# sandyz1000/face-landmark-detector

Measured on AMD Instinct MI355X. Metric: faces/sec (whole node), 256x256 batch inference: fused preprocess + FCN-8 forward + softmax + top-4 landmark decode + similarity/alignment warp, higher is better.
Workload: dtype f32; 1 GPU; BASELINE configs[1]: batch=64/GPU 256x256x3 uint8 crops, fcn_8(68) vanilla encoder fp32, random-init weights (seed 2), decode top-4 thresh 0, align to 256x256; global_batch=64, parallelism=dp1

## Files before the change

### face-landmark-detector_amd/build.py

```python
from __future__ import annotations

import concurrent.futures
import hashlib
import os
import shutil
import subprocess
import sys

HERE = os.path.dirname(os.path.abspath(__file__))
ROOT = os.path.dirname(HERE)
CSRC = os.path.join(HERE, "csrc")
INCLUDE = os.path.join(ROOT, "include")
OBJ_DIR = os.path.join(HERE, "csrc", "build")
LIB_PATH = os.path.join(HERE, "libflm_hip.so")

SOURCES = [
    "flm_api.hip",
    "flm_pack.hip",
    "flm_enc1.hip",
    "flm_igemm.hip",
    "flm_igemm_bf16.hip",
    "flm_conv3_halo.hip",
    "flm_score1x1.hip",
    "flm_tail_bf16.hip",
    "flm_convt.hip",
    "flm_up3_wreg.hip",
    "flm_decode.hip",
    "flm_decode_stats.hip",
    "flm_cand.hip",
    "flm_misc.hip",
    "flm_frames.hip",
    "flm_warp_fmt.hip",
    "flm_frames_nv12.hip",
    "flm_track.hip",
    "flm_track_assoc.hip",
    "flm_quality.hip",
    "flm_track_exit.hip",
    "flm_pose.hip",
    "flm_mobile.hip",
]
FLAGS = ["--offload-arch=gfx950", "-O3", "-fPIC", "-std=c++17", "-ffp-contract=off",
         "-Wall", "-Wno-unused-function", "-I", INCLUDE, "-I", CSRC]


FILE_FLAGS = {"flm_enc1.hip": ["-mllvm", "-amdgpu-mfma-vgpr-form"]}


def _hipcc() -> str:
    for c in (shutil.which("hipcc"), "/opt/rocm/bin/hipcc"):
        if c and os.path.exists(c):
            return c
    raise RuntimeError("hipcc not found: the HIP extension cannot be built")


def _stamp(paths) -> str:
    h = hashlib.sha256()
    h.update(" ".join(FLAGS).encode())
    h.update(repr(sorted(FILE_FLAGS.items())).encode())
    for p in sorted(paths):
        with open(p, "rb") as f:
            h.update(p.encode())
            h.update(f.read())
    return h.hexdigest()


def build(force: bool = False, verbose: bool = True, extra_flags=()) -> str:
    os.makedirs(OBJ_DIR, exist_ok=True)
    headers = [os.path.join(CSRC, f) for f in os.listdir(CSRC) if f.endswith(".h")] + \
              [os.path.join(INCLUDE, f) for f in os.listdir(INCLUDE) if f.endswith(".h")]
    srcs = [os.path.join(CSRC, s) for s in SOURCES]
    stamp = _stamp(srcs + headers) + " ".join(extra_flags)
    stamp_file = os.path.join(OBJ_DIR, "stamp.txt")
    if not force and os.path.exists(LIB_PATH) and os.path.exists(stamp_file) and open(stamp_file).read() == stamp:
        return LIB_PATH
    hipcc = _hipcc()

    def compile_one(src):
        obj = os.path.join(OBJ_DIR, os.path.basename(src) + ".o")
        cmd = [hipcc, *FLAGS, *FILE_FLAGS.get(os.path.basename(src), []), *extra_flags, "-c", src, "-o", obj]
        r = subprocess.run(cmd, capture_output=True, text=True)
        if r.returncode != 0:
            raise RuntimeError("hipcc failed on %s:\n%s\n%s" % (src, r.stdout, r.stderr))
        if verbose and r.stderr.strip():
            sys.stderr.write(r.stderr)
        return obj

    with concurrent.futures.ThreadPoolExecutor(max_workers=min(8, len(srcs))) as ex:
        objs = list(ex.map(compile_one, srcs))
    cmd = [hipcc, "--offload-arch=gfx950", "-shared", "-fPIC", "-o", LIB_PATH, *objs]
    r = subprocess.run(cmd, capture_output=True, text=True)
    if r.returncode != 0:
        raise RuntimeError("link failed:\n%s\n%s" % (r.stdout, r.stderr))
    with open(stamp_file, "w") as f:
        f.write(stamp)
    if verbose:
        print("built", LIB_PATH)
    return LIB_PATH


if __name__ == "__main__":
    build(force="--force" in sys.argv)
```

### face-landmark-detector_amd/csrc/flm_api.hip

```cpp
#include <cmath>
#include <cstdarg>
#include <cstdio>
#include <cstring>

#include "flm_common.h"

namespace flm {

static thread_local char g_err[512] = "";

void set_error(const char* fmt, ...) {
  va_list ap;
  va_start(ap, fmt);
  vsnprintf(g_err, sizeof(g_err), fmt, ap);
  va_end(ap);
}

int hip_fail(hipError_t e, const char* what) {
  set_error("HIP error %d (%s) at %s", (int)e, hipGetErrorString(e), what);
  return FLM_ERR_HIP;
}

struct Knob {
  const char* key;
  std::atomic<int> value;
  bool (*valid)(int);
  const char* domain;
};
static Knob g_knobs[] = {
    {"bf16_big_tiles", {1}, nullptr, nullptr},
    {"bf16_lds_dma", {1}, nullptr, nullptr},
    {"bf16_mfma16", {1}, nullptr, nullptr},
    {"bf16_halo_mfma16", {1}, nullptr, nullptr},
    {"f32_two_level", {1}, nullptr, nullptr},
    {"f32_lean_tile", {1}, nullptr, nullptr},
    {"bf16_group_n", {0}, [](int v) { return v >= 0 && v <= 32 && !(v & (v - 1)); }, "0 or a power of two <= 32"},
    {"bf16_conv3_halo", {1}, nullptr, nullptr},
    {"bf16_score1x1", {1}, nullptr, nullptr},
    {"bf16_fused_tail", {1}, nullptr, nullptr},
    {"decode_lds_dma", {1}, nullptr, nullptr},
    {"posmajor_order", {1}, nullptr, nullptr},
    {"warp_rows", {1}, [](int v) { return v == 0 || v == 1 || v == 4; }, "0, 1 or 4"},
    {"up3_cand8", {1}, [](int v) { return v >= 0 && v <= 7; }, "in [0,7]"},
    {"up3_cand8_rows", {0}, [](int v) { return v >= 0 && v <= 8 && !(v & (v - 1)); }, "0, 1, 2, 4 or 8"},
    {"up3_wreg", {0}, [](int v) { return v == 0 || v == 1; }, "0 or 1"},
    {"f32_fc6_rows", {0}, [](int v) { return v == 0 || v == 64 || v == 128; }, "0, 64 or 128"},
};
static_assert(sizeof(g_knobs) / sizeof(g_knobs[0]) == KNOB_COUNT, "one row per KnobId");
int tuning(KnobId id) { return g_knobs[id].value.load(std::memory_order_relaxed); }
static Knob* find_knob(const char* who, const char* key) {
  for (Knob& k : g_knobs)
    if (!strcmp(k.key, key)) return &k;
  set_error("%s: unknown key '%s'", who, key);
  return nullptr;
}

struct ProfRec {
  const char* name;
  hipEvent_t a, b;
};
static ProfRec* g_prof = nullptr;
static int g_prof_cap = 0, g_prof_n = 0;
static char g_prof_filter[32] = "";

struct ProfScope {
  hipStream_t s;
  ProfRec* r;
  ProfScope(hipStream_t st, const char* name) : s(st), r(nullptr) {
    if (name && g_prof && g_prof_n < g_prof_cap && (!g_prof_filter[0] || !strcmp(g_prof_filter, name))) {
      r = &g_prof[g_prof_n++];
      r->name = name;
      (void)hipEventRecord(r->a, s);
    }
  }
  ~ProfScope() {
    if (r) (void)hipEventRecord(r->b, s);
  }
};

struct CandOpts {
  int enable, sub, cap_div;
};
static bool resolve_opts(const flm_forward_opts* o, CandOpts* c) {
  c->enable = 1;
  c->sub = 0;
  c->cap_div = 1;
  if (!o) return true;
  if (o->struct_size < sizeof(flm_forward_opts)) {
    set_error("flm_forward_opts: struct_size %u is smaller than this library's %zu (initialise with flm_forward_opts_init)",
              o->struct_size, sizeof(flm_forward_opts));
    return false;
  }
  if (o->candidate_sub_phases < 0 || o->candidate_sub_phases > 16 || o->candidate_cap_div < 1) {
    set_error("flm_forward_opts: candidate_sub_phases must be in [0,16] and candidate_cap_div >= 1");
    return false;
  }
  c->enable = o->landmark_candidates != 0;
  c->sub = o->candidate_sub_phases;
  c->cap_div = o->candidate_cap_div;
  return true;
}
static int cand_sub_for(const CandOpts& c, int n_points, bool bf16) {
  if (c.sub > 0) return c.sub;
  return n_points <= 8 ? (bf16 ? 4 : 2) : (n_points <= 15 ? 6 : 8);
}
static bool landmark_candidates_enabled(const CandOpts& c, const ConvTGeom& g, int fcn32, int decode_mode, int n_points,
                                        int oh, int ow) {
  return c.enable && !fcn32 && decode_mode == FLM_DECODE_TOPN && n_points >= 1 && n_points <= 32 &&
         convt_candidates_supported(g) && (long long)oh * ow < (1 << 17);
}

struct EncNames {
  char s[kMaxEnc][8];
  EncNames() {
    for (int i = 0; i < kMaxEnc; ++i) snprintf(s[i], sizeof(s[i]), "enc%d", i + 1);
  }
};

static size_t take(size_t& cur, size_t bytes) {
  size_t o = cur;
  cur = align_up(cur + bytes, 256);
  return o;
}

Fcn8Ws fcn8_ws_layout(int n, int h, int w, int C, int dtype, int out_mode, int decode_mode, int n_points,
                      int arch, const flm_forward_opts* opts) {
  Fcn8Ws W;
  CandOpts co;
  if (!resolve_opts(opts, &co)) {
    W = Fcn8Ws();
    W.total = 0;
    return W;
// ... 44 lines not shown
    }
  }
  W.total = cur;
  return W;
}

static int check_dtype_classes(const char* what, int dtype, int C) {
  if (dtype != FLM_F32 && dtype != FLM_BF16) {
    set_error("%s: unknown dtype %d (FLM_F32 = 0, FLM_BF16 = 1)", what, dtype);
    return FLM_ERR_UNSUPPORTED;
  }
  if (C < 1 || C > kMaxClasses) {
    set_error("%s: n_classes must be in [1,%d] (got %d)", what, kMaxClasses, C);
    return FLM_ERR_SHAPE;
  }
  return FLM_OK;
}

static int check_fcn8_shape(int n, int h, int w, int C, int dtype) {
  const int rc = check_dtype_classes("fcn8", dtype, C);
  if (rc) return rc;
  if (n <= 0 || h <= 0 || w <= 0 || (h % 32) || (w % 32)) {
    set_error("fcn8: input must be [N>0, H, W, 3] with H and W multiples of 32 (got n=%d h=%d w=%d)", n, h, w);
    return FLM_ERR_SHAPE;
  }
  if (n > (1 << 24) || h > (1 << 15) || w > (1 << 15) || (long long)n * (h + 32) * (w + 32) * C >= (1ll << 40)) {
    set_error("fcn8: batch too large (n=%d h=%d w=%d: at most 2^40 output values per call)", n, h, w);
    return FLM_ERR_SHAPE;
  }
  return FLM_OK;
}

static int conv_layer(hipStream_t s, const char* blob, const ConvPack& c, const void* x, void* y, int n, int h,
                      int w, int relu, int pool, int posmajor, int dtype, int out_f32 = 0,
                      float* splitk_ws = nullptr, size_t splitk_bytes = 0, int stride = 1,
                      const void* res = nullptr) {
  IgemmDesc d;
  d.bf16 = dtype == FLM_BF16;
  d.out_f32 = out_f32;
  d.stride = stride;
  d.res = res;
  d.splitk_ws = splitk_ws;
  d.splitk_ws_bytes = splitk_bytes;
  d.x = x;
  d.wt = blob + c.w;
  d.scale = reinterpret_cast<const float*>(blob + c.scale);
  d.shift = reinterpret_cast<const float*>(blob + c.shift);
  d.y = y;
  d.n = n; d.h = h; d.w = w; d.cin = c.cin;
  d.cout = c.cout; d.coutpad = c.coutpad; d.ldc = c.cout;
  d.kh = c.kh; d.kw = c.kw; d.pad = c.pad;
  d.relu = relu; d.pool = pool; d.posmajor = posmajor;
  return launch_igemm(s, d);
}

static ConvTDesc up_desc(const Fcn8Pack& L, const char* blob, int layer, int n, int hi, int wi, const float* x, void* y) {
  ConvTDesc t;
  t.g = L.g;
  t.n = n; t.hi = hi; t.wi = wi;
  t.x = x; t.y = y;
  t.epilogue = 0;
  t.s = layer != 3 ? 2 : (L.spec.fcn32 ? 32 : 8);
  if (layer == 3) {
    t.wf = blob + L.up3; t.skip = nullptr;
    t.ho = t.s * hi + t.s; t.wo = t.s * wi + t.s; t.ldy = L.g.C;
  } else {
    t.wf = blob + (layer == 5 ? L.up5 : L.up4); t.skip = static_cast<const float*>(y);
    t.ho = 2 * hi; t.wo = 2 * wi; t.ldy = L.g.Cp;
  }
  return t;
}

}

using namespace flm;

extern "C" {

int flm_abi_version(void) { return FLM_ABI_VERSION; }

int flm_debug_query(const char* key, int arg) {
  if (key && !strcmp(key, "igemm_occupancy")) return igemm_occupancy((size_t)arg);
  if (key && !strcmp(key, "igemm_posmajor_rows")) return igemm_posmajor_rows_last();
  return -1;
}

int flm_set_tuning(const char* key, int value) {
  if (!key) return FLM_ERR_ARG;
  if (!strcmp(key, "none")) return FLM_OK;
  if (!strcmp(key, "landmark_candidates") || !strcmp(key, "candidate_sub_phases") || !strcmp(key, "candidate_cap_div")) {
    set_error("flm_set_tuning: '%s' changes the workspace layout and is a per-call option now: pass flm_forward_opts to "
              "flm_fcn_workspace_bytes_opts / flm_fcn_forward_opts", key);
    return FLM_ERR_ARG;
  }
  Knob* k = find_knob("flm_set_tuning", key);
  if (!k) return FLM_ERR_ARG;
  if (k->valid && !k->valid(value)) {
    set_error("flm_set_tuning: %s must be %s", key, k->domain);
    return FLM_ERR_ARG;
  }
  k->value.store(value, std::memory_order_relaxed);
  return FLM_OK;
}

int flm_get_tuning(const char* key, int* value) {
  if (!key || !value) {
    set_error("flm_get_tuning: null argument");
    return FLM_ERR_ARG;
  }
  const Knob* k = find_knob("flm_get_tuning", key);
  if (!k) return FLM_ERR_ARG;
  *value = k->value.load(std::memory_order_relaxed);
  return FLM_OK;
}

int flm_profile_enable(int max_records) {
  if (g_prof) return FLM_OK;
  if (max_records <= 0 || max_records > (1 << 20)) {
    set_error("flm_profile_enable: bad record count");
    return FLM_ERR_ARG;
  }
  g_prof = new ProfRec[max_records];
  for (int i = 0; i < max_records; ++i) {
    FLM_HIP(hipEventCreate(&g_prof[i].a));
    FLM_HIP(hipEventCreate(&g_prof[i].b));
  }
  g_prof_cap = max_records;
  g_prof_n = 0;
  return FLM_OK;
}

int flm_profile_reset(void) {
  g_prof_n = 0;
  return FLM_OK;
}

int flm_profile_read(int index, char* name_out, int name_cap, float* ms_out) {
  if (!g_prof || index < 0 || index >= g_prof_n) return 1;
  ProfRec& r = g_prof[index];
  FLM_HIP(hipEventSynchronize(r.b));
  FLM_HIP(hipEventElapsedTime(ms_out, r.a, r.b));
  if (name_out && name_cap > 0) {
    strncpy(name_out, r.name, name_cap - 1);
    name_out[name_cap - 1] = 0;
  }
  return FLM_OK;
}

int flm_profile_disable(void) {
  if (!g_prof) return FLM_OK;
  for (int i = 0; i < g_prof_cap; ++i) {
    (void)hipEventDestroy(g_prof[i].a);
    (void)hipEventDestroy(g_prof[i].b);
  }
  delete[] g_prof;
  g_prof = nullptr;
  g_prof_cap = g_prof_n = 0;
  return FLM_OK;
}
int flm_profile_filter(const char* layer) {
  if (layer && strlen(layer) >= sizeof(g_prof_filter)) {
    set_error("flm_profile_filter: layer name too long");
    return FLM_ERR_ARG;
  }
  strcpy(g_prof_filter, layer ? layer : "");
  return FLM_OK;
// ... 213 lines not shown
  void* fc6 = ws + W.fc6;
  void* fc7 = ws + W.fc7;
  float* score5 = reinterpret_cast<float*>(ws + W.score5);
  float* fuse4 = reinterpret_cast<float*>(ws + W.fuse4);
  float* seg = reinterpret_cast<float*>(ws + W.seg);

  const int h5 = h / 32, w5 = w / 32, h4 = h / 16, w4 = w / 16, h3 = h / 8, w3 = w / 8;
  const auto conv = [&](const char* name, const ConvPack& c, const void* x, void* y, int hh, int ww, int relu, int pool,
                        int posmajor, int out_f32, bool splitk) {
    ProfScope ps(s, name);
    return conv_layer(s, blob, c, x, y, n, hh, ww, relu, pool, posmajor, dtype, out_f32,
                      splitk ? reinterpret_cast<float*>(ws + W.splitk) : nullptr, splitk ? W.splitk_bytes : 0);
  };
  static const EncNames enc_name_table;
  const char (*enc_names)[8] = enc_name_table.s;
  int hs[kMaxEnc], wsz[kMaxEnc];
  enc_dims(A, h, w, hs, wsz);
  {
    int h8 = hs[A.f_idx[2]], h16 = hs[A.f_idx[3]], h32 = hs[A.f_idx[4]];
    if (h8 != h / 8 || h16 != h / 16 || h32 != h / 32) {
      set_error("flm_fcn_forward: encoder grid %d/%d/%d does not match the decoder's H/8, H/16, H/32", h8, h16, h32);
      return FLM_ERR_SHAPE;
    }
  }
  for (int i = 0; i < A.n_enc; ++i) {
    const EncLayer& e = A.enc[i];
    const int src = e.src >= 0 ? e.src : i - 1;
    const void* xin = src >= 0 ? static_cast<const void*>(ws + W.act[src]) : x_dev;
    const int hi = src >= 0 ? hs[src] : h, wi = src >= 0 ? wsz[src] : w;
    void* yout = ws + W.act[i];
    const float* w0 = reinterpret_cast<const float*>(blob + (i == 0 ? L.enc1_w : L.enc[i].w));
    const float* sc0 = reinterpret_cast<const float*>(blob + (i == 0 ? L.enc1_scale : L.enc[i].scale));
    const float* sh0 = reinterpret_cast<const float*>(blob + (i == 0 ? L.enc1_shift : L.enc[i].shift));
    ProfScope ps(s, enc_names[i]);
    switch (e.kind) {
      case ENC_FIRST3:
        rc = launch_enc1(s, xin, in_format, n, hi, wi, w0, sc0, sh0, yout, bf, e.pool);
        break;
      case ENC_MB_CONV1:
        rc = launch_mb_conv1(s, xin, in_format, n, hi, wi, w0, sc0, sh0, yout, bf);
        break;
      case ENC_RN_CONV1:
        rc = launch_rn_conv1(s, xin, in_format, n, hi, wi, w0, sc0, sh0, yout, bf);
        break;
      case ENC_MAXPOOL3:
        rc = launch_maxpool3(s, xin, n, hi, wi, e.cin, yout, bf);
        break;
      case ENC_MB_DW:
        rc = launch_mb_depthwise(s, xin, n, hi, wi, e.cin, e.stride, w0, sc0, sh0, yout, bf);
        break;
      case ENC_CONV3:
        rc = conv(nullptr, L.enc[i], xin, yout, hi, wi,  1, e.pool, 0, 0, true);
        break;
      case ENC_MB_PW:
        if (L.enc[i].cin != e.cin) {
          int pn = n, ph = hi, pw = wi;
          if (!(pw & 1)) pw >>= 1;
          else if (!(ph & 1)) ph >>= 1;
          else if (!(pn & 1)) pn >>= 1;
          else {
            set_error("flm_fcn_forward: the paired pointwise conv needs an even number of pixels per batch");
            rc = FLM_ERR_SHAPE;
            break;
          }
          rc = conv_layer(s, blob, L.enc[i], xin, yout, pn, ph, pw,  2, 0, 0, dtype);
        } else {
          rc = conv_layer(s, blob, L.enc[i], xin, yout, n, hi, wi,  2, 0, 0, dtype);
        }
        break;
      case ENC_CONV:
        rc = conv_layer(s, blob, L.enc[i], xin, yout, n, hi, wi, e.relu, 0, 0, dtype, 0, nullptr, 0, e.stride,
                        e.res >= 0 ? ws + W.act[e.res] : nullptr);
        break;
      default:
        set_error("flm_fcn_forward: unknown encoder layer kind %d", e.kind);
        rc = FLM_ERR_ARG;
    }
    if (rc) return rc;
  }
  if ((rc = conv("fc6", L.fc6, f[4], fc6, h5, w5, 1, 0,  1, 0, true))) return rc;
  if ((rc = conv("fc7", L.fc7, fc6, fc7, h5, w5, 1, 0, 0, 0, true))) return rc;
  if ((rc = conv("score5", L.score5, fc7, score5, h5, w5, 0, 0, 0,  1, true))) return rc;
  if (!fcn32) {
    if ((rc = conv("score4", L.score4, f[3], fuse4, h4, w4, 0, 0, 0, 1, false))) return rc;
    const auto score3 = [&] { return conv("score3", L.score3, f[2], seg, h3, w3, 0, 0, 0, 1, false); };
    const auto up5 = [&] {
      ProfScope ps(s, "up5");
      return launch_convt(s, up_desc(L, blob, 5, n, h5, w5, score5, fuse4));
    };
    const auto up4 = [&] {
      ProfScope ps(s, "up4");
      return launch_convt(s, up_desc(L, blob, 4, n, h4, w4, fuse4, seg));
    };
    if (!(bf && L.g.C == 68 && L.score3.cin == 256 && L.score3.kh == 1)) {
      if ((rc = score3()) || (rc = up5()) || (rc = up4())) return rc;
    } else {
      if ((rc = up5())) return rc;
      int fused;
      { ProfScope ps(s, "seg_fused");
        fused = launch_seg_fused_bf16(s, fuse4, blob + L.up4, f[2], blob + L.score3.w,
                                      reinterpret_cast<const float*>(blob + L.score3.scale),
                                      reinterpret_cast<const float*>(blob + L.score3.shift), seg, n, h4, w4, L.g.C, L.g.Cp,
                                      L.g.G, L.score3.cin, L.score3.coutpad); }
      if (fused < 0) return fused;
      if (!fused && ((rc = score3()) || (rc = up4()))) return rc;
    }
  }
  ConvTDesc t = fcn32 ? up_desc(L, blob, 3, n, h5, w5, score5, nullptr) : up_desc(L, blob, 3, n, h3, w3, seg, nullptr);
  if (out_mode == FLM_OUT_LOGITS || out_mode == FLM_OUT_PROBS) {
    t.y = out_dev;
    t.epilogue = (out_mode == FLM_OUT_PROBS) ? 1 : 0;
    if (out_mode == FLM_OUT_LOGITS && (C & 3)) {
      set_error("flm_fcn8_forward: FLM_OUT_LOGITS needs n_classes %% 4 == 0");
      return FLM_ERR_UNSUPPORTED;
    }
    ProfScope ps(s, "up3");
    return launch_convt(s, t);
  }
  if (out_mode == FLM_OUT_CLASSMAP) {
    t.y = out_dev;
    t.epilogue = 2;
    ProfScope ps(s, "up3");
    return launch_convt(s, t);
  }
  const int stats = out_mode == FLM_OUT_LANDMARKS_STATS;
  float* probs = reinterpret_cast<float*>(ws + W.probs);
  const unsigned* gate = nullptr;
  if (W.cand != SIZE_MAX) {
    float* sub = reinterpret_cast<float*>(ws + W.sub);
    float* tau = reinterpret_cast<float*>(ws + W.tau);
    unsigned* cnt = reinterpret_cast<unsigned*>(ws + W.cand_cnt);
    unsigned long long* cand = reinterpret_cast<unsigned long long*>(ws + W.cand);
    FLM_HIP(hipMemsetAsync(cnt, 0, sizeof(unsigned) * ((size_t)n + 1), s));
    ConvTDesc ts = t;
    ts.y = sub; ts.epilogue = 4; ts.sub = W.cand_sub;
    { ProfScope ps(s, "up3_sub");
    rc = launch_convt(s, ts); }
    if (rc) return rc;
    { ProfScope ps(s, "tau");
    rc = launch_cand_tau(s, reinterpret_cast<const unsigned*>(sub), n, convt_sample_slots(L.g, t.hi, t.wi, W.cand_sub), 16 * L.g.MT, C, n_points, tau); }
    if (rc) return rc;
    ConvTDesc tc = t;
    tc.y = nullptr; tc.epilogue = 3; tc.tau = tau; tc.cand = cand; tc.cand_cnt = cnt; tc.cand_cap = W.cand_cap;
    tc.scratch = probs; tc.scratch_bytes = sizeof(float) * (size_t)n * W.oh * W.ow * C;
    { ProfScope ps(s, "up3");
    rc = launch_convt(s, tc); }
    if (rc) return rc;
    { ProfScope ps(s, "decode");
    rc = launch_cand_merge(s, cand, cnt, n, W.ow, C, n_points, thresh, W.cand_cap, static_cast<double*>(out_dev), stats); }
    if (rc) return rc;
    gate = cnt + n;
    t.gate = gate;
  }
  t.y = probs;
  t.epilogue = 1;
  { ProfScope ps(s, gate ? "up3_fallback" : "up3");
  rc = launch_convt(s, t); }
  if (rc) return rc;
  ProfScope ps(s, gate ? "decode_fallback" : "decode");
  return launch_decode(s, probs, n, W.oh, W.ow, C, decode_mode, n_points, thresh,
                       static_cast<double*>(out_dev), ws + W.decode,
                       decode_ws_bytes(n, W.oh, W.ow, C, decode_mode, n_points, stats), gate, stats);
}

int flm_fcn8_run_layer(flm_stream_t stream, const void* packed_dev, const char* layer, const void* x_dev,
                       void* y_dev, int n, int h, int w, int C, int dtype) {
  if (!packed_dev || !layer || !x_dev || !y_dev || n <= 0 || h <= 0 || w <= 0) {
    set_error("flm_fcn8_run_layer: bad argument");
    return FLM_ERR_ARG;
  }
  if (check_dtype_classes("flm_fcn8_run_layer", dtype, C)) return FLM_ERR_UNSUPPORTED;
  const Fcn8Pack L = fcn8_pack_layout(C, dtype);
  const char* blob = static_cast<const char*>(packed_dev);
  hipStream_t s = static_cast<hipStream_t>(stream);
  if (!strncmp(layer, "enc", 3) && layer[3] >= '2' && layer[3] <= '5' && layer[4] == 0)
    return conv_layer(s, blob, L.enc[layer[3] - '1'], x_dev, y_dev, n, h, w, 1, 1, 0, dtype);
  if (!strcmp(layer, "fc6")) return conv_layer(s, blob, L.fc6, x_dev, y_dev, n, h, w, 1, 0, 1, dtype);
  if (!strcmp(layer, "fc7")) return conv_layer(s, blob, L.fc7, x_dev, y_dev, n, h, w, 1, 0, 0, dtype);
  if (!strcmp(layer, "score5")) return conv_layer(s, blob, L.score5, x_dev, y_dev, n, h, w, 0, 0, 0, dtype, 1);
  if (!strcmp(layer, "score4")) return conv_layer(s, blob, L.score4, x_dev, y_dev, n, h, w, 0, 0, 0, dtype, 1);
  if (!strcmp(layer, "score3")) return conv_layer(s, blob, L.score3, x_dev, y_dev, n, h, w, 0, 0, 0, dtype, 1);
  if (!strcmp(layer, "up5") || !strcmp(layer, "up4") || !strcmp(layer, "up3")) {
    if (layer[2] == '3' && (C & 3)) {
      set_error("flm_fcn8_run_layer: \"up3\" writes raw logits, which needs n_classes %% 4 == 0");
      return FLM_ERR_UNSUPPORTED;
    }
    return launch_convt(s, up_desc(L, blob, layer[2] - '0', n, h, w, static_cast<const float*>(x_dev), y_dev));
  }
  set_error("flm_fcn8_run_layer: unknown layer '%s'", layer);
// ... 1005 lines not shown
```

### face-landmark-detector_amd/csrc/flm_common.h

```cpp
#pragma once

#include <hip/hip_runtime.h>
#include <stddef.h>
#include <stdint.h>

#include <atomic>
#include <mutex>

#include "flm.h"

namespace flm {

void set_error(const char* fmt, ...);
int hip_fail(hipError_t e, const char* what);

#define FLM_HIP(call)                                            \
  do {                                                           \
    hipError_t e_ = (call);                                      \
    if (e_ != hipSuccess) return ::flm::hip_fail(e_, #call);     \
  } while (0)

#define FLM_LAUNCH_CHECK(what)                                   \
  do {                                                           \
    hipError_t e_ = hipGetLastError();                           \
// ... 26 lines not shown

constexpr int kFc = 4096;
constexpr int kMaxClasses = 96;
constexpr int kMaxEnc = 64;

enum EncKind {
  ENC_FIRST3 = 0,
  ENC_CONV3 = 1,
  ENC_MB_CONV1 = 2,
  ENC_MB_DW = 3,
  ENC_MB_PW = 4,
  ENC_RN_CONV1 = 5,
  ENC_MAXPOOL3 = 6,
  ENC_CONV = 7
};
struct EncLayer {
  int cin, cout, bn, pool;
  int kind, stride;
  int k, relu;
  int src, res;
};
struct ArchSpec {
  int n_enc;
  EncLayer enc[kMaxEnc];
  int f_idx[5];
  int fcn32;
  int valid;
};
void enc_dims(const ArchSpec& A, int h, int w, int* hs, int* ws);
inline int enc_has_params(const EncLayer& e) { return e.kind != ENC_MAXPOOL3; }
ArchSpec arch_spec(int arch);

struct ConvTGeom {
  int C;
  int Cp;
  int MT;
  int G;
  int bf16;
};
ConvTGeom convt_geom(int C, int dtype);

struct ConvPack {
  size_t w;
  size_t scale;
  size_t shift;
  int cin, cout, coutpad, kh, kw, pad;
};

struct Fcn8Pack {
  size_t enc1_w;
  size_t enc1_scale, enc1_shift;
  ConvPack enc[kMaxEnc];
  ConvPack fc6, fc7, score5, score4, score3;
  size_t up5, up4, up3;
  ConvTGeom g;
  int dtype;
  int arch;
  ArchSpec spec;
  size_t total;
};
Fcn8Pack fcn8_pack_layout(int C, int dtype, int arch = 0);

struct Fcn8Ws {
  size_t act[kMaxEnc];
  size_t f[5];
  size_t fc6, fc7, score5, fuse4, seg;
  size_t splitk;
  size_t splitk_bytes;
  size_t probs;
  size_t decode;
  size_t sub, tau, cand, cand_cnt;
  int cand_cap;
  int cand_sub;
  size_t total;
  int oh, ow;
};
Fcn8Ws fcn8_ws_layout(int n, int h, int w, int C, int dtype, int out_mode, int decode_mode, int n_points,
                      int arch = 0, const flm_forward_opts* opts = nullptr);

enum KnobId {
  KNOB_BF16_BIG_TILES, KNOB_BF16_LDS_DMA, KNOB_BF16_MFMA16, KNOB_BF16_HALO_MFMA16, KNOB_F32_TWO_LEVEL, KNOB_F32_LEAN_TILE,
  KNOB_BF16_GROUP_N, KNOB_BF16_CONV3_HALO, KNOB_BF16_SCORE1X1, KNOB_BF16_FUSED_TAIL, KNOB_DECODE_LDS_DMA,
  KNOB_POSMAJOR_ORDER, KNOB_WARP_ROWS, KNOB_UP3_CAND8, KNOB_UP3_CAND8_ROWS, KNOB_UP3_WREG, KNOB_F32_FC6_ROWS,
  KNOB_COUNT
};
int tuning(KnobId id);

int launch_pack_fcn(hipStream_t s, const flm_fcn_params& p, int C, const Fcn8Pack& L, char* blob);

int launch_enc1(hipStream_t s, const void* x, int in_format, int n, int h, int w, const float* w1p,
                const float* scale, const float* shift, void* f1, int out_bf16, int pool);

struct IgemmDesc {
  const void* x;
  const void* wt;
  const float* scale;
  const float* shift;
  void* y;
  int bf16;
  int out_f32;
  int n, h, w, cin;
  int cout;
  int coutpad;
  int ldc;
  int kh, kw, pad;
  int relu, pool, posmajor;
  int stride;
  const void* res;
  float* splitk_ws;
  size_t splitk_ws_bytes;
};
int launch_igemm(hipStream_t s, const IgemmDesc& d);
int igemm_occupancy(size_t lds_bytes);
int igemm_posmajor_rows_last();
int launch_seg_fused_bf16(hipStream_t s, const float* fuse4, const void* w4_packed, const void* f3, const void* w3,
                          const float* scale3, const float* shift3, float* seg, int n, int h4, int w4d, int C, int Cp,
                          int G, int cin3, int coutpad3);

struct ConvTDesc {
  const float* x;
  const void* wf;
  const float* skip;
  void* y;
  int n, hi, wi;
  int ho, wo;
  int s;
  int ldy;
  int epilogue;
  ConvTGeom g;
  int sub = 0;
  const float* tau = nullptr;
  unsigned long long* cand = nullptr;
  unsigned* cand_cnt = nullptr;
  int cand_cap = 0;
  const unsigned* gate = nullptr;
  void* scratch = nullptr;
  size_t scratch_bytes = 0;
};
int launch_convt(hipStream_t s, const ConvTDesc& d);
int convt_candidates_supported(const ConvTGeom& g);
__host__ __device__ inline int convt_share_layout(const ConvTGeom& g, int s) {
  return g.C == 68 && (g.bf16 ? g.G == 9 : g.G == 17) && (s % 4) == 0;
}
int convt_sample_slots(const ConvTGeom& g, int hi, int wi, int sub);
int launch_cand_tau(hipStream_t s, const unsigned* wave_max, int n, int slots, int ld, int l, int n_points, float* tau);

int launch_mb_conv1(hipStream_t s, const void* x, int in_format, int n, int h, int w, const float* wgt,
                    const float* scale, const float* shift, void* y, int bf16);
int launch_mb_depthwise(hipStream_t s, const void* x, int n, int h, int w, int c, int stride, const float* wgt,
                        const float* scale, const float* shift, void* y, int bf16);
int launch_rn_conv1(hipStream_t s, const void* x, int in_format, int n, int h, int w, const float* wgt,
                    const float* scale, const float* shift, void* y, int bf16);
int launch_maxpool3(hipStream_t s, const void* x, int n, int h, int w, int c, void* y, int bf16);

size_t decode_ws_bytes(int n, int h, int w, int l, int mode, int n_points, int stats = 0);
int launch_decode(hipStream_t s, const float* hm, int n, int h, int w, int l, int mode, int n_points, float thresh,
                  double* out, void* ws, size_t ws_bytes, const unsigned* gate = nullptr, int stats = 0);
size_t decode_sweep_ws_bytes(int n, int h, int w, int l, const int* modes, int n_modes);
int launch_decode_sweep(hipStream_t s, const float* hm, int n, int h, int w, int l, const int* modes, int n_modes,
                        float thresh, double* out, void* ws, size_t ws_bytes);
int launch_gaussian_heatmaps(hipStream_t s, const double* kp, int n, int l, int h, int w, double two_sigma_sq,
                             float* out);
int launch_cand_merge(hipStream_t s, const unsigned long long* cand, unsigned* cand_cnt, int n, int w, int l,
                      int n_points, float thresh, int cap, double* out, int stats = 0);

int launch_preprocess(hipStream_t s, const uint8_t* img, int n, int h, int w, int norm, float* out);
int launch_similarity(hipStream_t s, const double* lm, const double* tmpl, int n, int k, double sx, double sy, float* m);
int launch_similarity_weighted(hipStream_t s, const double* lm, size_t lm_stride, const double* wt, size_t w_stride,
                               const double* tmpl, int n, int k, double sx, double sy, float* m);
int launch_warp(hipStream_t s, const void* src, int src_is_u8, int n, int hs, int ws, const float* m, float* dst,
                int hd, int wd);
int launch_crop_resize(hipStream_t s, const uint8_t* frame, int fh, int fw, const int32_t* boxes, int k,
                       uint8_t* out, int oh, int ow, const int32_t* frame_idx = nullptr, size_t frame_stride = 0,
                       int nframes = 0);
int launch_landmarks_to_frame(hipStream_t s, const double* lm, const int32_t* boxes, int k, int c, int grid_h,
                              int grid_w, int fh, int fw, double* out);
int launch_warp_frames(hipStream_t s, const uint8_t* frames, size_t frame_stride, int nframes, int fh, int fw,
                       const int32_t* frame_idx, const int32_t* boxes, const float* m, int k, float* dst, int hd,
                       int wd, int samples);
int launch_warp_fmt(hipStream_t s, const void* src, int src_is_u8, int n, int hs, int ws, const float* m, void* dst, int hd,
                    int wd, const flm_image_format* fmt);
int launch_warp_frames_fmt(hipStream_t s, const uint8_t* frames, size_t frame_stride, int nframes, int fh, int fw,
                           const int32_t* frame_idx, const int32_t* boxes, const float* m, int k, void* dst, int hd,
                           int wd, int samples, const flm_image_format* fmt);

int launch_frames_to_bgr_nv12(hipStream_t s, const uint8_t* frames, size_t frame_stride, int nframes, int fh, int fw,
                              const flm_frame_format* src, uint8_t* out);
int launch_crop_resize_nv12(hipStream_t s, const uint8_t* frames, size_t frame_stride, int nframes, int fh, int fw,
                            const int32_t* boxes, const int32_t* frame_idx, int k, uint8_t* out, int oh, int ow,
                            const flm_frame_format* src);
int launch_warp_frames_nv12(hipStream_t s, const uint8_t* frames, size_t frame_stride, int nframes, int fh, int fw,
                            const int32_t* frame_idx, const int32_t* boxes, const float* m, int k, void* dst, int hd,
                            int wd, int samples, const flm_image_format* fmt, const flm_frame_format* src);
size_t nv12_format_bytes(const char* who, const flm_frame_format* src, int fh, int fw);

int launch_track_seed(hipStream_t s, const int32_t* boxes, int k, int in_h, int in_w, int fh, int fw, float* m,
                      int32_t* status);
int launch_landmarks_from_crop(hipStream_t s, const double* lm, size_t lm_stride, const float* m, int k, int c, double sx,
                               double sy, double* out);
int launch_track_step(hipStream_t s, const char* who, const double* lm, size_t lm_stride, const double* wt, size_t w_stride,
// ... 92 lines not shown
```

Measured before the change: 7846 faces/s.

## Fuse fp32 FCN-8 tail score-conv, upsample and skip-add into single kernels

Adds fp32 fused kernels that compute each FCN-8 tail stage (2x transposed-conv upsample of the coarser score plus the 1x1 score conv on the skip feature, with scale/shift) in one pass. One kernel covers fuse4 and one covers seg, and both are enabled by default through a new knob. The 1x1 weights are staged in LDS, and results are combined in a per-wave LDS tile before a coalesced store. This removes the separate score4/score3 and up5/up4 launches and the intermediate round-trips through global memory. In exchange it uses a large LDS footprint with one block per CU, and the kernels are specialised to C=68 and K=256.

```diff
diff --git a/face-landmark-detector_amd/build.py b/face-landmark-detector_amd/build.py
--- a/face-landmark-detector_amd/build.py
+++ b/face-landmark-detector_amd/build.py
@@ -23,6 +23,7 @@
     "flm_conv3_halo.hip",
     "flm_score1x1.hip",
     "flm_tail_bf16.hip",
+    "flm_tail_f32.hip",
     "flm_convt.hip",
     "flm_up3_wreg.hip",
     "flm_decode.hip",
diff --git a/face-landmark-detector_amd/csrc/flm_api.hip b/face-landmark-detector_amd/csrc/flm_api.hip
--- a/face-landmark-detector_amd/csrc/flm_api.hip
+++ b/face-landmark-detector_amd/csrc/flm_api.hip
@@ -45,9 +45,11 @@
     {"up3_cand8_rows", {0}, [](int v) { return v >= 0 && v <= 8 && !(v & (v - 1)); }, "0, 1, 2, 4 or 8"},
     {"up3_wreg", {0}, [](int v) { return v == 0 || v == 1; }, "0 or 1"},
     {"f32_fc6_rows", {0}, [](int v) { return v == 0 || v == 64 || v == 128; }, "0, 64 or 128"},
+    {"f32_fused_tail", {3}, [](int v) { return v >= 0 && v <= 3; }, "in [0,3]"},
 };
 static_assert(sizeof(g_knobs) / sizeof(g_knobs[0]) == KNOB_COUNT, "one row per KnobId");
 int tuning(KnobId id) { return g_knobs[id].value.load(std::memory_order_relaxed); }
+static std::atomic<int> g_fused_tail_last{0};
 static Knob* find_knob(const char* who, const char* key) {
   for (Knob& k : g_knobs)
     if (!strcmp(k.key, key)) return &k;
@@ -258,6 +260,7 @@
 int flm_debug_query(const char* key, int arg) {
   if (key && !strcmp(key, "igemm_occupancy")) return igemm_occupancy((size_t)arg);
   if (key && !strcmp(key, "igemm_posmajor_rows")) return igemm_posmajor_rows_last();
+  if (key && !strcmp(key, "fused_tail_stages")) return g_fused_tail_last.load(std::memory_order_relaxed);
   return -1;
 }
 
@@ -637,7 +640,7 @@
   if ((rc = conv("fc7", L.fc7, fc6, fc7, h5, w5, 1, 0, 0, 0, true))) return rc;
   if ((rc = conv("score5", L.score5, fc7, score5, h5, w5, 0, 0, 0,  1, true))) return rc;
   if (!fcn32) {
-    if ((rc = conv("score4", L.score4, f[3], fuse4, h4, w4, 0, 0, 0, 1, false))) return rc;
+    const auto score4 = [&] { return conv("score4", L.score4, f[3], fuse4, h4, w4, 0, 0, 0, 1, false); };
     const auto score3 = [&] { return conv("score3", L.score3, f[2], seg, h3, w3, 0, 0, 0, 1, false); };
     const auto up5 = [&] {
       ProfScope ps(s, "up5");
@@ -647,19 +650,40 @@
       ProfScope ps(s, "up4");
       return launch_convt(s, up_desc(L, blob, 4, n, h4, w4, fuse4, seg));
     };
-    if (!(bf && L.g.C == 68 && L.score3.cin == 256 && L.score3.kh == 1)) {
-      if ((rc = score3()) || (rc = up5()) || (rc = up4())) return rc;
+    const auto cscale = [&](const ConvPack& c) { return reinterpret_cast<const float*>(blob + c.scale); };
+    const auto cshift = [&](const ConvPack& c) { return reinterpret_cast<const float*>(blob + c.shift); };
+    const int ran_fused = bf ? 0 : tail_f32_stages(L.g, L.score4, L.score3, n, h5, w5);
+    if (ran_fused) {
+      if (ran_fused & 2) {
+        ProfScope ps(s, "fuse4_fused");
+        rc = launch_fuse4_fused_f32(s, score5, blob + L.up5, f[3], blob + L.score4.w, cscale(L.score4), cshift(L.score4),
+                                    fuse4, n, h5, w5);
+      } else {
+        (void)((rc = score4()) || (rc = up5()));
+      }
+      if (rc) return rc;
+      if (ran_fused & 1) {
+        ProfScope ps(s, "seg_fused");
+        rc = launch_seg_fused_f32(s, fuse4, blob + L.up4, f[2], blob + L.score3.w, cscale(L.score3), cshift(L.score3), seg, n,
+                                  h4, w4);
+      } else {
+        (void)((rc = score3()) || (rc = up4()));
+      }
+      if (rc) return rc;
+    } else if (!(bf && L.g.C == 68 && L.score3.cin == 256 && L.score3.kh == 1)) {
+      if ((rc = score4()) || (rc = score3()) || (rc = up5()) || (rc = up4())) return rc;
     } else {
-      if ((rc = up5())) return rc;
+      if ((rc = score4()) || (rc = up5())) return rc;
       int fused;
       { ProfScope ps(s, "seg_fused");
-        fused = launch_seg_fused_bf16(s, fuse4, blob + L.up4, f[2], blob + L.score3.w,
-                                      reinterpret_cast<const float*>(blob + L.score3.scale),
-                                      reinterpret_cast<const float*>(blob + L.score3.shift), seg, n, h4, w4, L.g.C, L.g.Cp,
-                                      L.g.G, L.score3.cin, L.score3.coutpad); }
+        fused = launch_seg_fused_bf16(s, fuse4, blob + L.up4, f[2], blob + L.score3.w, cscale(L.score3), cshift(L.score3), seg,
+                                      n, h4, w4, L.g.C, L.g.Cp, L.g.G, L.score3.cin, L.score3.coutpad); }
       if (fused < 0) return fused;
       if (!fused && ((rc = score3()) || (rc = up4()))) return rc;
     }
+    g_fused_tail_last.store(ran_fused, std::memory_order_relaxed);
+  } else {
+    g_fused_tail_last.store(0, std::memory_order_relaxed);
   }
   ConvTDesc t = fcn32 ? up_desc(L, blob, 3, n, h5, w5, score5, nullptr) : up_desc(L, blob, 3, n, h3, w3, seg, nullptr);
   if (out_mode == FLM_OUT_LOGITS || out_mode == FLM_OUT_PROBS) {
diff --git a/face-landmark-detector_amd/csrc/flm_common.h b/face-landmark-detector_amd/csrc/flm_common.h
--- a/face-landmark-detector_amd/csrc/flm_common.h
+++ b/face-landmark-detector_amd/csrc/flm_common.h
@@ -132,7 +132,7 @@
   KNOB_BF16_BIG_TILES, KNOB_BF16_LDS_DMA, KNOB_BF16_MFMA16, KNOB_BF16_HALO_MFMA16, KNOB_F32_TWO_LEVEL, KNOB_F32_LEAN_TILE,
   KNOB_BF16_GROUP_N, KNOB_BF16_CONV3_HALO, KNOB_BF16_SCORE1X1, KNOB_BF16_FUSED_TAIL, KNOB_DECODE_LDS_DMA,
   KNOB_POSMAJOR_ORDER, KNOB_WARP_ROWS, KNOB_UP3_CAND8, KNOB_UP3_CAND8_ROWS, KNOB_UP3_WREG, KNOB_F32_FC6_ROWS,
-  KNOB_COUNT
+  KNOB_F32_FUSED_TAIL, KNOB_COUNT
 };
 int tuning(KnobId id);
 
@@ -166,6 +166,11 @@
 int launch_seg_fused_bf16(hipStream_t s, const float* fuse4, const void* w4_packed, const void* f3, const void* w3,
                           const float* scale3, const float* shift3, float* seg, int n, int h4, int w4d, int C, int Cp,
                           int G, int cin3, int coutpad3);
+int tail_f32_stages(const ConvTGeom& g, const ConvPack& score4, const ConvPack& score3, int n, int h5, int w5);
+int launch_fuse4_fused_f32(hipStream_t s, const float* score5, const void* w5_packed, const void* f4, const void* w4c,
+                           const float* scale4, const float* shift4, float* fuse4, int n, int h5, int w5d);
+int launch_seg_fused_f32(hipStream_t s, const float* fuse4, const void* w4_packed, const void* f3, const void* w3,
+                         const float* scale3, const float* shift3, float* seg, int n, int h4, int w4d);
 
 struct ConvTDesc {
   const float* x;
diff --git a/face-landmark-detector_amd/csrc/flm_tail_f32.hip b/face-landmark-detector_amd/csrc/flm_tail_f32.hip
--- /dev/null
+++ b/face-landmark-detector_amd/csrc/flm_tail_f32.hip
@@ -0,0 +1,269 @@
+#include "flm_convt_dev.h"
+
+namespace flm {
+
+typedef float f32x16_t3 __attribute__((ext_vector_type(16)));
+
+constexpr int T3_C = 68, T3_K = 256, T3_STEPS = T3_K / 32, T3_G = 17, T3_MT = 5, T3_SUBG = 6;
+constexpr int T3_WFULL_F4 = 2 * T3_STEPS * 4 * 64;
+constexpr int T3_W_F4 = T3_WFULL_F4 + T3_STEPS * 4 * 2 * 4;
+constexpr int T3_IMG = 32 * T3_C;
+constexpr int T3_WAVES = 8;
+constexpr int T3_WD = 2;
+constexpr int T3_PF = 3;
+
+__device__ __forceinline__ void tail_fused_f32_body(const float* __restrict__ x,
+                                                    const float4* __restrict__ wt,
+                                                    const float* __restrict__ feat,
+                                                    const float* __restrict__ wc,
+                                                    const float* __restrict__ scale, const float* __restrict__ shift,
+                                                    float* __restrict__ y,
+                                                    int n, int hi, int wi, int aw) {
+  extern __shared__ __attribute__((aligned(16))) char smem_raw[];
+  float4* ldsw = reinterpret_cast<float4*>(smem_raw);
+  float* img_all = reinterpret_cast<float*>(ldsw + T3_W_F4);
+  const int tid = threadIdx.x, nwaves = aw;
+  const int wave = __builtin_amdgcn_readfirstlane(tid >> 6);
+  const int phase = blockIdx.x & 3, a0 = phase >> 1, b0 = phase & 1;
+  const int wb = blockIdx.x >> 2, nbp = gridDim.x >> 2;
+  constexpr int kFill = (T3_C * (T3_K / 4) + 64 * T3_WAVES - 1) / (64 * T3_WAVES);
+  float4 wv[kFill];
+#pragma unroll
+  for (int it = 0; it < kFill; ++it) {
+    const int i = tid + it * 64 * T3_WAVES;
+    wv[it] = *reinterpret_cast<const float4*>(wc + 4 * (size_t)min(i, T3_C * (T3_K / 4) - 1));
+  }
+#pragma unroll
+  for (int it = 0; it < kFill; ++it) {
+    const int i = tid + it * 64 * T3_WAVES;
+    const int row = i >> 6, c4 = i & 63;
+    const int st = c4 >> 3, t = (c4 >> 1) & 3, h = c4 & 1;
+    const int dst = row < 64 ? (((row >> 5) * T3_STEPS + st) * 4 + t) * 64 + h * 32 + (row & 31)
+                             : T3_WFULL_F4 + ((st * 4 + t) * 2 + h) * 4 + (row - 64);
+    if (i < T3_C * (T3_K / 4)) ldsw[dst] = wv[it];
+  }
+  __syncthreads();
+  const int hw = hi * wi, P = n * hw, slices = (P + 31) >> 5;
+  const int ho = 2 * hi, wo = 2 * wi;
+  const f32x4 zero4 = (f32x4){0.f, 0.f, 0.f, 0.f};
+
+  for (int sl = wave < nwaves ? wb * nwaves + wave : slices; sl < slices; sl += nbp * nwaves) {
+    int lane = tid & 63;
+    asm volatile("" : "+v"(lane));
+    const int r16 = lane & 15, lr = lane & 31, lh = lane >> 5;
+    float* im = img_all + wave * T3_IMG;
+    const float4* wph = wt + (size_t)phase * (T3_G * T3_MT * 64) + lane;
+    const float* frow;
+    {
+      const int p = sl * 32 + lr, pp = p < P ? p : P - 1;
+      const int f = pp / hw, rem = pp - f * hw, i0 = rem / wi, j0 = rem - i0 * wi;
+      frow = feat + (((size_t)f * ho + (2 * i0 + a0)) * wo + (2 * j0 + b0)) * T3_K + 4 * lh;
+    }
+    float4 fa[T3_STEPS][4];
+#pragma unroll
+    for (int st = 0; st < T3_PF; ++st)
+#pragma unroll
+      for (int t = 0; t < 4; ++t) fa[st][t] = *reinterpret_cast<const float4*>(frow + 32 * st + 8 * t);
+#pragma unroll 1
+    for (int nt = 0; nt < 2; ++nt) {
+      int q = lane >> 4;
+      asm volatile("" : "+v"(q));
+      const int p = sl * 32 + nt * 16 + r16;
+      const bool pv = p < P;
+      const int pp = pv ? p : P - 1;
+      const int f = pp / hw, rem = pp - f * hw, i0 = rem / wi, j0 = rem - i0 * wi;
+      float4 xf[T3_G];
+#pragma unroll
+      for (int g = 0; g < T3_G; ++g) {
+        const int k0 = 16 * g + 4 * q;
+        const int tap = k0 / T3_C, c = k0 - tap * T3_C;
+        const int ii = i0 - (tap >> 1), jj = j0 - (tap & 1);
+        const bool ok = pv && ii >= 0 && jj >= 0;
+        const size_t off = ok ? (((size_t)f * hi + ii) * wi + jj) * T3_C + c : 0;
+        const float4 v = *reinterpret_cast<const float4*>(x + off);
+        xf[g] = make_float4(ok ? v.x : 0.f, ok ? v.y : 0.f, ok ? v.z : 0.f, ok ? v.w : 0.f);
+      }
+      f32x4 acc[T3_MT], tmp[T3_MT];
+#pragma unroll
+      for (int m = 0; m < T3_MT; ++m) acc[m] = tmp[m] = zero4;
+      const float4* wp = wph;
+      asm volatile("" : "+v"(wp));
+      float4 afr[T3_WD + 1][T3_MT];
+#pragma unroll
+      for (int g = 0; g < T3_WD; ++g)
+#pragma unroll
+        for (int m = 0; m < T3_MT; ++m) afr[g][m] = wp[(g * T3_MT + m) * 64];
+#pragma unroll
+      for (int g = 0; g < T3_G; ++g) {
+        if (g + T3_WD < T3_G) {
+#pragma unroll
+          for (int m = 0; m < T3_MT; ++m) afr[(g + T3_WD) % (T3_WD + 1)][m] = wp[((g + T3_WD) * T3_MT + m) * 64];
+        }
+        const float4* af = afr[g % (T3_WD + 1)];
+        if (g < T3_SUBG) {
+#pragma unroll
+          for (int m = 0; m < T3_MT; ++m) acc[m] = __builtin_amdgcn_mfma_f32_16x16x4f32(af[m].x, xf[g].x, acc[m], 0, 0, 0);
+#pragma unroll
+          for (int m = 0; m < T3_MT; ++m) acc[m] = __builtin_amdgcn_mfma_f32_16x16x4f32(af[m].y, xf[g].y, acc[m], 0, 0, 0);
+#pragma unroll
+          for (int m = 0; m < T3_MT; ++m) acc[m] = __builtin_amdgcn_mfma_f32_16x16x4f32(af[m].z, xf[g].z, acc[m], 0, 0, 0);
+#pragma unroll
+          for (int m = 0; m < T3_MT; ++m) acc[m] = __builtin_amdgcn_mfma_f32_16x16x4f32(af[m].w, xf[g].w, acc[m], 0, 0, 0);
+        } else {
+          const bool sub_first = g % T3_SUBG == 0;
+          const bool sub_last = g == T3_G - 1 || (g + 1) % T3_SUBG == 0;
+#pragma unroll
+          for (int m = 0; m < T3_MT; ++m)
+            tmp[m] = __builtin_amdgcn_mfma_f32_16x16x4f32(af[m].x, xf[g].x, sub_first ? zero4 : tmp[m], 0, 0, 0);
+#pragma unroll
+          for (int m = 0; m < T3_MT; ++m) tmp[m] = __builtin_amdgcn_mfma_f32_16x16x4f32(af[m].y, xf[g].y, tmp[m], 0, 0, 0);
+#pragma unroll
+          for (int m = 0; m < T3_MT; ++m) tmp[m] = __builtin_amdgcn_mfma_f32_16x16x4f32(af[m].z, xf[g].z, tmp[m], 0, 0, 0);
+#pragma unroll
+          for (int m = 0; m < T3_MT; ++m) tmp[m] = __builtin_amdgcn_mfma_f32_16x16x4f32(af[m].w, xf[g].w, tmp[m], 0, 0, 0);
+          if (sub_last) {
+#pragma unroll
+            for (int m = 0; m < T3_MT; ++m) acc[m] += tmp[m];
+          }
+        }
+        __builtin_amdgcn_sched_barrier(0);
+      }
+      float* ip = im + (nt * 16 + r16) * T3_C;
+#pragma unroll
+      for (int m = 0; m < 4; ++m)
+        *reinterpret_cast<float4*>(ip + 16 * m + 4 * q) = make_float4(acc[m][0], acc[m][1], acc[m][2], acc[m][3]);
+      ip[64 + q] = acc[4][0];
+    }
+    __builtin_amdgcn_wave_barrier();
+    {
+      f32x16_t3 acc[3], sum[3], top[3];
+      const f32x16_t3 zero16 = {0.f, 0.f, 0.f, 0.f, 0.f, 0.f, 0.f, 0.f, 0.f, 0.f, 0.f, 0.f, 0.f, 0.f, 0.f, 0.f};
+      const float4* wl01 = ldsw + lane;
+      const float4* wl2 = ldsw + T3_WFULL_F4 + lh * 4 + (lr & 3);
+#pragma unroll
+      for (int st = 0; st < T3_STEPS; ++st) {
+        if (st + T3_PF < T3_STEPS) {
+#pragma unroll
+          for (int t = 0; t < 4; ++t) fa[st + T3_PF][t] = *reinterpret_cast<const float4*>(frow + 32 * (st + T3_PF) + 8 * t);
+        }
+        if (st > 0) {
+#pragma unroll
+          for (int j = 0; j < 3; ++j) {
+            if (st & 1) sum[j] = acc[j] + 0.f;
+            else sum[j] += acc[j];
+            asm volatile("" : "+v"(sum[j]));
+          }
+        }
+#pragma unroll
+        for (int t = 0; t < 4; ++t) {
+          const float4 b0 = wl01[((0 * T3_STEPS + st) * 4 + t) * 64], b1 = wl01[((1 * T3_STEPS + st) * 4 + t) * 64],
+                       b2 = wl2[(st * 4 + t) * 8];
+          const float4 av = fa[st][t];
+          acc[0] = __builtin_amdgcn_mfma_f32_32x32x2f32(av.x, b0.x, t == 0 ? zero16 : acc[0], 0, 0, 0);
+          acc[1] = __builtin_amdgcn_mfma_f32_32x32x2f32(av.x, b1.x, t == 0 ? zero16 : acc[1], 0, 0, 0);
+          acc[2] = __builtin_amdgcn_mfma_f32_32x32x2f32(av.x, b2.x, t == 0 ? zero16 : acc[2], 0, 0, 0);
+          acc[0] = __builtin_amdgcn_mfma_f32_32x32x2f32(av.y, b0.y, acc[0], 0, 0, 0);
+          acc[1] = __builtin_amdgcn_mfma_f32_32x32x2f32(av.y, b1.y, acc[1], 0, 0, 0);
+          acc[2] = __builtin_amdgcn_mfma_f32_32x32x2f32(av.y, b2.y, acc[2], 0, 0, 0);
+          acc[0] = __builtin_amdgcn_mfma_f32_32x32x2f32(av.z, b0.z, acc[0], 0, 0, 0);
+          acc[1] = __builtin_amdgcn_mfma_f32_32x32x2f32(av.z, b1.z, acc[1], 0, 0, 0);
+          acc[2] = __builtin_amdgcn_mfma_f32_32x32x2f32(av.z, b2.z, acc[2], 0, 0, 0);
+          acc[0] = __builtin_amdgcn_mfma_f32_32x32x2f32(av.w, b0.w, acc[0], 0, 0, 0);
+          acc[1] = __builtin_amdgcn_mfma_f32_32x32x2f32(av.w, b1.w, acc[1], 0, 0, 0);
+          acc[2] = __builtin_amdgcn_mfma_f32_32x32x2f32(av.w, b2.w, acc[2], 0, 0, 0);
+        }
+        if (st > 0 && (st & 1) == 0) {
+#pragma unroll
+          for (int j = 0; j < 3; ++j) {
+            if (st == 2) top[j] = sum[j] + 0.f;
+            else top[j] += sum[j];
+          }
+        }
+        __builtin_amdgcn_sched_barrier(0);
+      }
+#pragma unroll
+      for (int j = 0; j < 3; ++j) {
+        const f32x16_t3 res = top[j] + (sum[j] + acc[j]);
+        const int c = 32 * j + lr;
+        if (c < T3_C) {
+          const float scj = scale[c], shj = shift[c];
+#pragma unroll
+          for (int r = 0; r < 16; ++r) {
+            float* ip = im + ((r & 3) + 8 * (r >> 2) + 4 * lh) * T3_C + c;
+            *ip = *ip + fmaf(res[r], scj, shj);
+          }
+        }
+      }
+    }
+    __builtin_amdgcn_wave_barrier();
+    const int npx = min(32, P - sl * 32);
+    for (int i = lane; i < npx * (T3_C / 4); i += 64) {
+      const int pl = i / (T3_C / 4), f4 = i - pl * (T3_C / 4);
+      const int p = sl * 32 + pl;
+      const int f = p / hw, rem = p - f * hw, i0 = rem / wi, j0 = rem - i0 * wi;
+      float* d = y + (((size_t)f * ho + (2 * i0 + a0)) * wo + (2 * j0 + b0)) * T3_C + 4 * f4;
+      *reinterpret_cast<float4*>(d) = *reinterpret_cast<const float4*>(im + pl * T3_C + 4 * f4);
+    }
+    __builtin_amdgcn_wave_barrier();
+  }
+}
+
+__global__ __launch_bounds__(64 * T3_WAVES, 1) void seg_fused_f32_kernel(const float* __restrict__ fuse4, const float4* __restrict__ w4,
+                                                                         const float* __restrict__ f3, const float* __restrict__ w3,
+                                                                         const float* __restrict__ scale3, const float* __restrict__ shift3,
+                                                                         float* __restrict__ seg, int n, int h4, int w4d, int aw) {
+  tail_fused_f32_body(fuse4, w4, f3, w3, scale3, shift3, seg, n, h4, w4d, aw);
+}
+
+__global__ __launch_bounds__(64 * T3_WAVES, 1) void fuse4_fused_f32_kernel(const float* __restrict__ score5, const float4* __restrict__ w5,
+                                                                           const float* __restrict__ f4, const float* __restrict__ w4c,
+                                                                           const float* __restrict__ scale4, const float* __restrict__ shift4,
+                                                                           float* __restrict__ fuse4, int n, int h5, int w5d, int aw) {
+  tail_fused_f32_body(score5, w5, f4, w4c, scale4, shift4, fuse4, n, h5, w5d, aw);
+}
+
+static bool tail_f32_covers(const ConvTGeom& g, const ConvPack& c, int n, int hi, int wi) {
+  return !g.bf16 && g.C == T3_C && g.Cp == T3_C && g.G == T3_G && g.MT == T3_MT && c.cin == T3_K && c.cout == T3_C &&
+         c.coutpad >= T3_C && c.kh == 1 && c.kw == 1 && c.pad == 0 && tuning(KNOB_F32_TWO_LEVEL) != 0 && n >= 1 && hi >= 1 &&
+         wi >= 1 && (long long)n * hi * wi < (1ll << 28);
+}
+
+template <class K>
+static int launch_tail_f32(hipStream_t s, K kernel, FuncAttrOnce& attr, const char* what, const float* x, const void* wt,
+                           const void* feat, const void* wc, const float* scale, const float* shift, float* y, int n, int hi,
+                           int wi) {
+  const int slices = (n * hi * wi + 31) / 32;
+  int waves = (slices + 63) / 64;
+  if (waves > T3_WAVES) waves = T3_WAVES;
+  int per_phase = (slices + waves - 1) / waves;
+  if (per_phase > 64) per_phase = 64;
+    constexpr size_t lds_max = sizeof(float4) * T3_W_F4 + sizeof(float) * (size_t)T3_WAVES * T3_IMG;
+  static_assert(lds_max <= 160 * 1024, "fused fp32 tail: LDS budget of a CU");
+  FLM_FUNC_ATTR_ONCE(attr, kernel, lds_max);
+  kernel<<<dim3((unsigned)(4 * per_phase)), 64 * T3_WAVES, lds_max, s>>>(x, static_cast<const float4*>(wt), static_cast<const float*>(feat),
+                                                                  static_cast<const float*>(wc), scale, shift, y, n, hi, wi, waves);
+  FLM_LAUNCH_CHECK(what);
+  return FLM_OK;
+}
+
+int tail_f32_stages(const ConvTGeom& g, const ConvPack& score4, const ConvPack& score3, int n, int h5, int w5) {
+  const int knob = tuning(KNOB_F32_FUSED_TAIL);
+  return ((knob & 1) && tail_f32_covers(g, score3, n, 2 * h5, 2 * w5) ? 1 : 0) |
+         ((knob & 2) && tail_f32_covers(g, score4, n, h5, w5) ? 2 : 0);
+}
+
+int launch_fuse4_fused_f32(hipStream_t s, const float* score5, const void* w5_packed, const void* f4, const void* w4c,
+                           const float* scale4, const float* shift4, float* fuse4, int n, int h5, int w5d) {
+  static FuncAttrOnce attr;
+  return launch_tail_f32(s, &fuse4_fused_f32_kernel, attr, "fuse4_fused_f32_kernel", score5, w5_packed, f4, w4c, scale4, shift4,
+                         fuse4, n, h5, w5d);
+}
+
+int launch_seg_fused_f32(hipStream_t s, const float* fuse4, const void* w4_packed, const void* f3, const void* w3,
+                         const float* scale3, const float* shift3, float* seg, int n, int h4, int w4d) {
+  static FuncAttrOnce attr;
+  return launch_tail_f32(s, &seg_fused_f32_kernel, attr, "seg_fused_f32_kernel", fuse4, w4_packed, f3, w3, scale3, shift3, seg, n,
+                         h4, w4d);
+}
+
+}
```

New measurement: 7904 faces/s, median of 6. No clear change (+0.7%).
